# vincentfung13/MINE

Measured on AMD Instinct MI355X. Metric: train imgs/sec (whole node) RealEstate10K 384x256 N=64, higher is better.
Workload: dtype bf16; 1 GPU; model=monodepth2-resnet50-mpi, global_batch=4, seq_len=64, parallelism=dp1, img_h=256, img_w=384, n_planes=64

## Files before the change

mine_amd/ops/bn.py:

```python
from __future__ import annotations

import torch
import torch.nn as nn
import torch.nn.functional as F

from mine_amd.ops.backend import get_extension, is_deterministic

_ACT = {"none": 0, "relu": 1, "lrelu": 2, "elu": 3, "add_relu": 4}


class _BNActFn(torch.autograd.Function):
    @staticmethod
    def forward(ctx, x_flat, res_flat, mean, invstd, gamma, beta, M, C, act,
                sync):
        ext = get_extension(required=True)
        y = ext.bn_act_fwd(x_flat, res_flat, mean, invstd,
                           gamma, beta, M, C, act)
        ctx.save_for_backward(x_flat, res_flat, mean, invstd, gamma, beta)
        ctx.geom = (M, C, act, sync)
        ctx.det = is_deterministic()
        return y

    @staticmethod
    def backward(ctx, gy):
        ext = get_extension(required=True)
        x_flat, res_flat, mean, invstd, gamma, beta = ctx.saved_tensors
        M, C, act, sync = ctx.geom
        gy = gy.contiguous()
        red = ext.bn_act_bwd_reduce(x_flat, res_flat, gy, mean, invstd,
                                    gamma, beta, M, C, act, 0, ctx.det)
        dbeta, dgamma = red[:C], red[C:]
        M_norm = M
        if sync:
            dbeta, dgamma = dbeta.clone(), dgamma.clone()
            torch.distributed.all_reduce(red)
            M_norm = M * torch.distributed.get_world_size()
        dx, dres = ext.bn_act_bwd_dx(x_flat, res_flat, gy, mean, invstd,
                                     gamma, beta, red, M, C, act, M_norm)
        return (dx, dres if act == _ACT["add_relu"] else None, None, None,
                dgamma, dbeta, None, None, None, None)


class _JoinStatsFn(torch.autograd.Function):

    @staticmethod
    def forward(ctx, y_dec, y_base, bias, B, S):
        ext = get_extension(required=True)
        det = is_deterministic()
        _, K, H, W = y_dec.shape
        x_flat, sums = ext.bn_join_stats(
            y_dec.permute(0, 2, 3, 1).reshape(-1),
            y_base.permute(0, 2, 3, 1).reshape(-1),
            bias.contiguous(), B, S, H * W, K, 0, det)
        ctx.geom = (B, S, H, W, K)
        ctx.det = det
        ctx.mark_non_differentiable(sums)
        return x_flat.view(B * S, H, W, K).permute(0, 3, 1, 2), sums

    @staticmethod
    def backward(ctx, g, _gsums):
        B, S, H, W, K = ctx.geom
        g_nhwc = g.permute(0, 2, 3, 1)
        g_base = g_nhwc.reshape(B, S, H, W, K).sum(1).permute(0, 3, 1, 2)
        return g, g_base, g_nhwc.sum((1, 2)), None, None

# ... 43 lines not shown
    def forward(self, x: torch.Tensor, res: torch.Tensor = None,
                sums: torch.Tensor = None):
        assert (res is not None) == (self.act == "add_relu")
        use_kernel = (
            x.is_cuda and x.dim() == 4
            and x.dtype in (torch.float32, torch.bfloat16, torch.float16)
            and x.is_contiguous(memory_format=torch.channels_last)
            and (res is None or (res.dtype == x.dtype and res.is_contiguous(
                memory_format=torch.channels_last)))
            and (self.training or not torch.is_grad_enabled()))
        if not use_kernel:
            return self._fallback(x, res)

        ext = get_extension(required=True)
        B, C, H, W = x.shape
        M = B * H * W
        x_flat = x.permute(0, 2, 3, 1).reshape(-1)
        res_flat = res.permute(0, 2, 3, 1).reshape(-1) if res is not None \
            else torch.empty(0, device=x.device, dtype=x.dtype)

        do_sync = self.training and self.sync and \
            torch.distributed.is_initialized() and \
            torch.distributed.get_world_size() > 1
        if self.training:
            if self.num_batches_tracked is not None:
                self.num_batches_tracked.add_(1)
            mom = self.momentum if self.momentum is not None else \
                1.0 / float(self.num_batches_tracked)
            track = self.track_running_stats and self.running_mean is not None
            empty = torch.empty(0, device=x.device, dtype=torch.float32)
            if do_sync:
                if sums is None:
                    sums = ext.bn_sums(x_flat.detach(), M, C, 0,
                                       is_deterministic())
                torch.distributed.all_reduce(sums)
                Mg = M * torch.distributed.get_world_size()
                mean = sums[:C] / Mg
                var = (sums[C:] / Mg - mean * mean).clamp_min_(0.0)
                invstd = torch.rsqrt(var + self.eps)
                if track:
                    with torch.no_grad():
                        self.running_mean += mom * (mean - self.running_mean)
                        unbiased = var * Mg / max(Mg - 1, 1)
                        self.running_var += mom * (unbiased - self.running_var)
                mean = mean.contiguous()
                invstd = invstd.contiguous()
# ... 24 lines not shown
```

mine_amd/ops/csrc/bindings.hip:

```cpp

#include <torch/extension.h>
#include <ATen/hip/HIPContext.h>
#include <c10/hip/HIPException.h>
#include <hip/hip_runtime.h>

#include <algorithm>
#include <array>
#include <climits>
#include <string>
#include <vector>

#include "launchers.h"

namespace {

hipStream_t stream() {
  return at::hip::getCurrentHIPStreamMasqueradingAsCUDA().stream();
}


constexpr unsigned kF32 = 1u << kElemF32;
constexpr unsigned kBF16 = 1u << kElemBF16;
constexpr unsigned kF16 = 1u << kElemF16;
constexpr unsigned k16 = kBF16 | kF16;
// ... 595 lines not shown
  const auto scaled = M_norm != M ? red * ((double)M / (double)M_norm) : red;
  auto dx = at::empty_like(x);
  auto dres = add_relu ? at::empty_like(x) : at::empty({0}, x.options());
  launched(who, mine_bn_act_bwd_dx(
                    x.data_ptr(), add_relu ? res_p : nullptr, gy.data_ptr(),
                    mean.data_ptr<float>(), invstd.data_ptr<float>(),
                    gamma.data_ptr<float>(), beta.data_ptr<float>(),
                    scaled.data_ptr<float>(), dx.data_ptr(),
                    add_relu ? dres.data_ptr() : nullptr, M, (int)C, (int)act,
                    (int)max_blocks, elem_of(x.scalar_type(), who), stream()));
  return {dx, dres};
}

std::vector<at::Tensor> bn_act_bwd(at::Tensor x, at::Tensor res,
                                   at::Tensor gy, at::Tensor mean,
                                   at::Tensor invstd, at::Tensor gamma,
                                   at::Tensor beta, int64_t M, int64_t C,
                                   int64_t act, bool deterministic) {
  auto red = bn_act_bwd_reduce(x, res, gy, mean, invstd, gamma, beta,
                               M, C, act, 0, deterministic);
  auto dxr = bn_act_bwd_dx(x, res, gy, mean, invstd, gamma, beta, red,
                           M, C, act, M, 0);
  return {dxr[0], dxr[1], red.narrow(0, C, C), red.narrow(0, 0, C)};
}


at::Tensor mpi_head_fwd(at::Tensor z, int64_t N, bool alpha) {
  const char* who = "mpi_head_fwd";
  check_arg(who, "z", z, z, kFloat, N * 4);
  TORCH_CHECK(N > 0, who, ": N must be positive");
  auto out = at::empty({N * 4}, z.options().dtype(at::kFloat));
  launched(who, mine_mpi_head_fwd(z.data_ptr(), out.data_ptr<float>(), N,
                                  alpha ? 1 : 0, elem_of(z.scalar_type(), who),
                                  stream()));
  return out;
}

at::Tensor mpi_head_bwd(at::Tensor z, at::Tensor gout, int64_t N, bool alpha) {
  const char* who = "mpi_head_bwd";
  check_arg(who, "z", z, z, kFloat, N * 4);
  check_arg(who, "gout", gout, z, kF32, N * 4);
  TORCH_CHECK(N > 0, who, ": N must be positive");
  auto gz = at::empty_like(z);
  launched(who, mine_mpi_head_bwd(z.data_ptr(), gout.data_ptr<float>(),
                                  gz.data_ptr(), N, alpha ? 1 : 0,
                                  elem_of(z.scalar_type(), who), stream()));
// ... 378 lines not shown
  mod.def("bn_join_stats", &bn_join_stats,
          "x = (y_base + bias) + y_dec with its per-channel (sum, sumsq)",
          py::arg("y_dec"), py::arg("y_base"), py::arg("bias"), py::arg("B"),
          py::arg("S"), py::arg("HW"), py::arg("C"),
          py::arg("max_blocks") = 0, py::arg("deterministic") = false);
  mod.def("bn_act_fwd", &bn_act_fwd, "fused normalize + activation",
          py::arg("x"), py::arg("res"), py::arg("mean"), py::arg("invstd"),
          py::arg("gamma"), py::arg("beta"), py::arg("M"), py::arg("C"),
          py::arg("act"), py::arg("max_blocks") = 0);
  mod.def("bn_act_bwd", &bn_act_bwd,
          "fused BN+act backward -> dx, dres, dgamma, dbeta", py::arg("x"),
          py::arg("res"), py::arg("gy"), py::arg("mean"), py::arg("invstd"),
          py::arg("gamma"), py::arg("beta"), py::arg("M"), py::arg("C"),
          py::arg("act"), py::arg("deterministic") = false);
  mod.def("bn_act_bwd_reduce", &bn_act_bwd_reduce, py::arg("x"),
          py::arg("res"), py::arg("gy"), py::arg("mean"), py::arg("invstd"),
          py::arg("gamma"), py::arg("beta"), py::arg("M"), py::arg("C"),
          py::arg("act"), py::arg("max_blocks") = 0,
          py::arg("deterministic") = false);
  mod.def("bn_act_bwd_dx", &bn_act_bwd_dx, py::arg("x"), py::arg("res"),
          py::arg("gy"), py::arg("mean"), py::arg("invstd"), py::arg("gamma"),
          py::arg("beta"), py::arg("red"), py::arg("M"), py::arg("C"),
          py::arg("act"), py::arg("M_norm"), py::arg("max_blocks") = 0);
  mod.def("mpi_head_fwd", &mpi_head_fwd,
          "dispconv out -> packed fp32 MPI (sigmoid rgb, |x|+1e-4 sigma)");
  mod.def("mpi_head_bwd", &mpi_head_bwd);
  mod.def("conv3x3_fwd", &conv3x3_fwd,
          "fused reflect/zero-pad + 3x3 conv on MFMA 16x16x32 tiles",
          py::arg("x_flat"), py::arg("wp"), py::arg("bias"), py::arg("out"),
          py::arg("N"), py::arg("H"), py::arg("W"), py::arg("C"), py::arg("K"),
          py::arg("pad_mode"), py::arg("src_h"), py::arg("src_w"),
          py::arg("off"), py::arg("c_mem") = 0);
  mod.def("conv3x3_pack", &conv3x3_pack,
          "gather a conv weight into MFMA fragment order (bf16 or fp16)",
          py::arg("w_flat"), py::arg("lut"), py::arg("dtype") = py::none());
  mod.def("conv3x3_wrw", &conv3x3_wrw,
          "reflect-pad 3x3 conv weight gradient, fp32 (K, C, 3, 3)",
          py::arg("x_flat"), py::arg("gy_flat"), py::arg("N"), py::arg("H"),
          py::arg("W"), py::arg("C"), py::arg("K"), py::arg("max_slabs") = 0);
  mod.def("conv3x3_wrw_bias", &conv3x3_wrw_bias,
          "weight and bias gradient in one pass -> (dw, db)",
          py::arg("x_flat"), py::arg("gy_flat"), py::arg("N"), py::arg("H"),
          py::arg("W"), py::arg("C"), py::arg("K"), py::arg("max_slabs") = 0);
}
```

mine_amd/ops/csrc/bn_kernels.hip:

```cpp

#include <hip/hip_runtime.h>
#include <hip/hip_bf16.h>
#include <cstdint>

#include "launchers.h"

namespace {

constexpr int kBlock = 256;

enum Act : int { ACT_NONE = 0, ACT_RELU = 1, ACT_LRELU = 2, ACT_ELU = 3,
                 ACT_ADD_RELU = 4 };

template <int ACT>
__device__ __forceinline__ float act_fwd_t(float z) {
  if constexpr (ACT == ACT_RELU || ACT == ACT_ADD_RELU)
    return z > 0.0f ? z : 0.0f;
  else if constexpr (ACT == ACT_LRELU)
    return z > 0.0f ? z : 0.1f * z;
  else if constexpr (ACT == ACT_ELU)
    return z > 0.0f ? z : __expf(z) - 1.0f;
  else
    return z;
}
// ... 80 lines not shown
#pragma unroll
    for (int j = 0; j < V; ++j) {
      if constexpr (DET) {
        s_a[threadIdx.x * V + j] = a[j];
        s_b[threadIdx.x * V + j] = b[j];
      } else {
        atomicAdd(&s_a[lm.lane_cv * V + j], a[j]);
        atomicAdd(&s_b[lm.lane_cv * V + j], b[j]);
      }
    }
  }
  __syncthreads();
  if constexpr (DET) {
    det_block_flush(s_a, s_b, cgv * V, lm.rows_per_blk(), lm.ncv * V, out, C,
                    lm.c0v * V);
  } else {
    for (int i = threadIdx.x; i < lm.ncv * V; i += kBlock) {
      atomicAdd(&out[lm.c0v * V + i], s_a[i]);
      atomicAdd(&out[C + lm.c0v * V + i], s_b[i]);
    }
  }
}

template <typename T, int V, bool DET>
__global__ void __launch_bounds__(kBlock)
bn_stats_vec_kernel(const void* __restrict__ x, float* __restrict__ sums,
                    int64_t M, int C, int cgv) {
  using Vec = BnVec<T, V>;
  bn_reduce<V, DET, int>(
      C, cgv, sums, [&](const auto& lm, float (&acc)[V], float (&asq)[V]) {
        const int Cv = C / V;
        const Vec* xv = static_cast<const Vec*>(x);
        const int rstride = lm.rstride();
        for (int64_t m = lm.row0(); m < M; m += rstride) {
          const Vec val = xv[m * Cv + lm.col()];
#pragma unroll
          for (int j = 0; j < V; ++j) {
            const float f = (float)val.v[j];
            acc[j] += f;
            asq[j] += f * f;
          }
        }
      });
}

__device__ __forceinline__ void bn_finalize_channel(
    float sum, float sumsq, int c, float* __restrict__ mean,
    float* __restrict__ invstd, float* __restrict__ running_mean,
    float* __restrict__ running_var, int64_t M, float eps, float momentum) {
  const float mu = sum / (float)M;
  float var = sumsq / (float)M - mu * mu;
  var = var > 0.0f ? var : 0.0f;
  mean[c] = mu;
  invstd[c] = rsqrtf(var + eps);
  if (running_mean) {
    running_mean[c] += momentum * (mu - running_mean[c]);
    const float unbiased = M > 1 ? var * (float)M / (float)(M - 1) : var;
    running_var[c] += momentum * (unbiased - running_var[c]);
  }
}

__global__ void bn_finalize_kernel(const float* __restrict__ sums,
                                   float* __restrict__ mean,
                                   float* __restrict__ invstd,
                                   float* __restrict__ running_mean,
                                   float* __restrict__ running_var,
                                   int64_t M, int C, float eps,
                                   float momentum) {
  const int c = blockIdx.x * kBlock + threadIdx.x;
  if (c >= C) return;
  bn_finalize_channel(sums[c], sums[C + c], c, mean, invstd, running_mean,
                      running_var, M, eps, momentum);
}

__global__ void __launch_bounds__(kBlock)
bn_det_finish_kernel(const float* __restrict__ ws, int G, int C, int cw,
                     float* __restrict__ out, float* __restrict__ mean,
                     float* __restrict__ invstd,
                     float* __restrict__ running_mean,
                     float* __restrict__ running_var, int64_t M, float eps,
                     float momentum) {
  __shared__ float s_a[kBlock], s_b[kBlock];
// ... 22 lines not shown
    for (; g < G; g += np, row += step) {
      a += row[0];
      b += row[C];
    }
  }
  s_a[threadIdx.x] = a;
  s_b[threadIdx.x] = b;
  __syncthreads();
  if (threadIdx.x >= cw || c >= C) return;
  float ta = 0.0f, tb = 0.0f;
  for (int q = 0; q < np; ++q) {
    ta += s_a[q * cw + lane_c];
    tb += s_b[q * cw + lane_c];
  }
  if (out) {
    out[c] = ta;
    out[C + c] = tb;
  }
  if (mean)
    bn_finalize_channel(ta, tb, c, mean, invstd, running_mean, running_var, M,
                        eps, momentum);
}

template <typename T, int V, int ACT, bool DET>
__global__ void __launch_bounds__(kBlock)
bn_act_bwd_reduce_vec_kernel(const void* __restrict__ x,
                             const void* __restrict__ res,
                             const void* __restrict__ gy,
                             const float* __restrict__ mean,
                             const float* __restrict__ invstd,
                             const float* __restrict__ gamma,
                             const float* __restrict__ beta,
                             float* __restrict__ out,
                             int64_t M, int C, int cgv) {
  using Vec = BnVec<T, V>;
  bn_reduce<V, DET, int>(
      C, cgv, out, [&](const auto& lm, float (&db)[V], float (&dg)[V]) {
        const int Cv = C / V;
        const int cb = lm.col() * V;
        float mu[V], is[V], ga[V], be[V];
#pragma unroll
        for (int j = 0; j < V; ++j) {
          mu[j] = mean[cb + j];
          is[j] = invstd[cb + j];
          ga[j] = gamma[cb + j];
          be[j] = beta[cb + j];
        }
        const Vec* xv = static_cast<const Vec*>(x);
        const Vec* gv = static_cast<const Vec*>(gy);
        const Vec* rv = static_cast<const Vec*>(res);
        const int rstride = lm.rstride();
        for (int64_t m = lm.row0(); m < M; m += rstride) {
          const int64_t off = m * Cv + lm.col();
          const Vec xval = xv[off];
          const Vec gval = gv[off];
          Vec rval;
          if constexpr (ACT == ACT_ADD_RELU) rval = rv[off];
#pragma unroll
          for (int j = 0; j < V; ++j) {
            const float xh = ((float)xval.v[j] - mu[j]) * is[j];
            float z = xh * ga[j] + be[j];
            if constexpr (ACT == ACT_ADD_RELU) z += (float)rval.v[j];
            const float g = (float)gval.v[j] * act_grad_t<ACT>(z);
            db[j] += g;
            dg[j] += g * xh;
          }
        }
      });
}


template <typename T, int V, bool DET>
__global__ void __launch_bounds__(kBlock)
bn_join_stats_vec_kernel(const void* __restrict__ y_dec,
                         const void* __restrict__ y_base,
                         const void* __restrict__ bias, void* __restrict__ x,
                         float* __restrict__ sums,
                         int64_t M, int HW, int S, int C, int cgv) {
  using Vec = BnVec<T, V>;
  bn_reduce<V, DET, int64_t>(
      C, cgv, sums, [&](const auto& lm, float (&acc)[V], float (&asq)[V]) {
        const int Cv = C / V;
        const Vec* dv = static_cast<const Vec*>(y_dec) + lm.col();
        const Vec* bv = static_cast<const Vec*>(y_base) + lm.col();
        const Vec* pv = static_cast<const Vec*>(bias) + lm.col();
        Vec* xv = static_cast<Vec*>(x) + lm.col();
        const int64_t row0 = lm.row0();
        const int rstride = lm.rstride();
        const int dq = rstride / HW, dr = rstride % HW;
// ... 14 lines not shown
            out.v[j] = xo;
            const float f = (float)xo;
            acc[j] += f;
            asq[j] += f * f;
          }
          xv[m * Cv] = out;
          p += dr;
          const int carry = p >= HW ? 1 : 0;
          p -= carry ? HW : 0;
          bs += dq + carry;
          s += dq_s + carry;
          b += dq_b;
          if (s >= S) {
            s -= S;
            ++b;
          }
        }
      });
}


constexpr int fwd_unroll(int act) { return act == ACT_ADD_RELU ? 1 : 3; }
constexpr int dx_unroll(int act) { return act == ACT_ADD_RELU ? 1 : 2; }

template <typename T, int V, int ACT>
__device__ __forceinline__ BnVec<T, V> bn_fwd_vec(
    const BnVec<T, V>& xval, const BnVec<T, V>& rval, const float (&mu)[V],
    const float (&is)[V], const float (&ga)[V], const float (&be)[V]) {
  BnVec<T, V> out;
#pragma unroll
  for (int j = 0; j < V; ++j) {
    float z = ((float)xval.v[j] - mu[j]) * is[j] * ga[j] + be[j];
    if constexpr (ACT == ACT_ADD_RELU) z += (float)rval.v[j];
    out.v[j] = (T)act_fwd_t<ACT>(z);
  }
  return out;
}

template <typename T, int V, int ACT, int U>
__global__ void __launch_bounds__(kBlock)
bn_act_fwd_vec_kernel(const void* __restrict__ x, const void* __restrict__ res,
                      const float* __restrict__ mean,
                      const float* __restrict__ invstd,
                      const float* __restrict__ gamma,
                      const float* __restrict__ beta, void* __restrict__ y,
                      int64_t M, int C, int cgv) {
  using Vec = BnVec<T, V>;
  const int Cv = C / V;
  const LaneMap<int64_t, int64_t> lm(Cv, cgv);
  if (!lm.active()) return;
  const int cb = lm.col() * V;
  float mu[V], is[V], ga[V], be[V];
#pragma unroll
  for (int j = 0; j < V; ++j) {
    mu[j] = mean[cb + j];
    is[j] = invstd[cb + j];
    ga[j] = gamma[cb + j];
    be[j] = beta[cb + j];
  }
  const Vec* xv = static_cast<const Vec*>(x) + lm.col();
  const Vec* rv = static_cast<const Vec*>(res) + lm.col();
  Vec* yv = static_cast<Vec*>(y) + lm.col();
  const int64_t rstride = lm.rstride();
  const int64_t step = rstride * Cv;
  int64_t m = lm.row0();
  int64_t off = lm.row0() * Cv;
  for (; m + (U - 1) * rstride < M; m += U * rstride, off += U * step) {
    Vec xval[U], rval[U];
#pragma unroll
    for (int u = 0; u < U; ++u) xval[u] = xv[off + u * step];
    if constexpr (ACT == ACT_ADD_RELU) {
#pragma unroll
      for (int u = 0; u < U; ++u) rval[u] = rv[off + u * step];
    }
#pragma unroll
    for (int u = 0; u < U; ++u)
      yv[off + u * step] =
          bn_fwd_vec<T, V, ACT>(xval[u], rval[u], mu, is, ga, be);
  }
// ... 2 lines not shown
    Vec rval;
    if constexpr (ACT == ACT_ADD_RELU) rval = rv[off];
    yv[off] = bn_fwd_vec<T, V, ACT>(xval, rval, mu, is, ga, be);
  }
}

template <typename T, int V, int ACT>
__device__ __forceinline__ void bn_dx_vec(
    const BnVec<T, V>& xval, const BnVec<T, V>& rval, const BnVec<T, V>& gval,
    const float (&mu)[V], const float (&is)[V], const float (&ga)[V],
    const float (&be)[V], const float (&r0)[V], const float (&r1)[V],
    float invM, BnVec<T, V>& dxo, BnVec<T, V>& dro) {
#pragma unroll
  for (int j = 0; j < V; ++j) {
    const float xh = ((float)xval.v[j] - mu[j]) * is[j];
    float z = xh * ga[j] + be[j];
    if constexpr (ACT == ACT_ADD_RELU) z += (float)rval.v[j];
    const float g = (float)gval.v[j] * act_grad_t<ACT>(z);
    if constexpr (ACT == ACT_ADD_RELU) dro.v[j] = (T)g;
    dxo.v[j] = (T)(ga[j] * is[j] * (g - (r0[j] + xh * r1[j]) * invM));
  }
}

template <typename T, int V, int ACT, int U>
__global__ void __launch_bounds__(kBlock)
bn_act_bwd_dx_vec_kernel(const void* __restrict__ x,
                         const void* __restrict__ res,
                         const void* __restrict__ gy,
                         const float* __restrict__ mean,
                         const float* __restrict__ invstd,
                         const float* __restrict__ gamma,
                         const float* __restrict__ beta,
                         const float* __restrict__ red,
                         void* __restrict__ dx, void* __restrict__ dres,
                         int64_t M, int C, int cgv) {
  using Vec = BnVec<T, V>;
  const int Cv = C / V;
  const float invM = 1.0f / (float)M;
  const LaneMap<int64_t, int64_t> lm(Cv, cgv);
  if (!lm.active()) return;
  const int cb = lm.col() * V;
  float mu[V], is[V], ga[V], be[V], r0[V], r1[V];
#pragma unroll
  for (int j = 0; j < V; ++j) {
    mu[j] = mean[cb + j];
    is[j] = invstd[cb + j];
    ga[j] = gamma[cb + j];
    be[j] = beta[cb + j];
    r0[j] = red[cb + j];
    r1[j] = red[C + cb + j];
  }
  const Vec* xv = static_cast<const Vec*>(x) + lm.col();
  const Vec* rv = static_cast<const Vec*>(res) + lm.col();
  const Vec* gv = static_cast<const Vec*>(gy) + lm.col();
  Vec* dxv = static_cast<Vec*>(dx) + lm.col();
  Vec* drv = static_cast<Vec*>(dres) + lm.col();
  const int64_t rstride = lm.rstride();
  const int64_t step = rstride * Cv;
  int64_t m = lm.row0();
  int64_t off = lm.row0() * Cv;
  for (; m + (U - 1) * rstride < M; m += U * rstride, off += U * step) {
    Vec xval[U], gval[U], rval[U];
#pragma unroll
    for (int u = 0; u < U; ++u) {
      xval[u] = xv[off + u * step];
      gval[u] = gv[off + u * step];
    }
    if constexpr (ACT == ACT_ADD_RELU) {
#pragma unroll
      for (int u = 0; u < U; ++u) rval[u] = rv[off + u * step];
    }
#pragma unroll
    for (int u = 0; u < U; ++u) {
// ... 60 lines not shown
  BN_VEC_SWITCH(
      T, C, return (int)grid_rows_v(M, Cv, cgv, kMaxGridReduce, max_blocks).x)
}

template <typename T, bool DET>
void launch_bn_stats(const void* x, float* sums, int64_t M, int C,
                     int max_blocks, hipStream_t s) {
  BN_VEC_SWITCH(
      T, C,
      hipLaunchKernelGGL(
          (bn_stats_vec_kernel<T, V, DET>),
          grid_rows_v(M, Cv, cgv, kMaxGridReduce, max_blocks), dim3(kBlock), 0,
          s, x, sums, M, C, cgv))
}

template <typename T>
void launch_bn_act_fwd(const void* x, const void* res, const float* mean,
                       const float* invstd, const float* gamma,
                       const float* beta, void* y, int64_t M, int C, int act,
                       int max_blocks, hipStream_t s) {
#define BN_LAUNCH(A)                                                          \
  hipLaunchKernelGGL((bn_act_fwd_vec_kernel<T, V, A, fwd_unroll(A)>),         \
                     grid_rows_v(M, Cv, cgv, kMaxGridStream, max_blocks),     \
                     dim3(kBlock), 0, s, x, res, mean, invstd, gamma, beta, y, \
                     M, C, cgv)
  BN_VEC_SWITCH(T, C, BN_ACT_SWITCH(act, BN_LAUNCH))
#undef BN_LAUNCH
}

template <typename T, bool DET>
void launch_bn_act_bwd_reduce(const void* x, const void* res, const void* gy,
                              const float* mean, const float* invstd,
                              const float* gamma, const float* beta,
                              float* out, int64_t M, int C, int act,
                              int max_blocks, hipStream_t s) {
#define BN_LAUNCH(A)                                                       \
  hipLaunchKernelGGL((bn_act_bwd_reduce_vec_kernel<T, V, A, DET>),         \
                     grid_rows_v(M, Cv, cgv, kMaxGridReduce, max_blocks),  \
                     dim3(kBlock), 0, s, x, res, gy, mean, invstd, gamma,  \
                     beta, out, M, C, cgv)
  BN_VEC_SWITCH(T, C, BN_ACT_SWITCH(act, BN_LAUNCH))
#undef BN_LAUNCH
}

template <typename T>
void launch_bn_act_bwd_dx(const void* x, const void* res, const void* gy,
                          const float* mean, const float* invstd,
                          const float* gamma, const float* beta,
                          const float* red, void* dx, void* dres, int64_t M,
                          int C, int act, int max_blocks, hipStream_t s) {
#define BN_LAUNCH(A)                                                        \
  hipLaunchKernelGGL((bn_act_bwd_dx_vec_kernel<T, V, A, dx_unroll(A)>),     \
                     grid_rows_v(M, Cv, cgv, kMaxGridStream, max_blocks),   \
                     dim3(kBlock), 0, s, x, res, gy, mean, invstd, gamma,   \
                     beta, red, dx, dres, M, C, cgv)
  BN_VEC_SWITCH(T, C, BN_ACT_SWITCH(act, BN_LAUNCH))
#undef BN_LAUNCH
}

template <typename T, bool DET>
void launch_bn_join_stats(const void* y_dec, const void* y_base,
                          const void* bias, void* x, float* sums, int64_t M,
                          int HW, int S, int C, int max_blocks,
                          hipStream_t s) {
  BN_VEC_CASE(
      8, C,
      hipLaunchKernelGGL(
          (bn_join_stats_vec_kernel<T, V, DET>),
          grid_rows_v(M, Cv, cgv, kMaxGridReduce, max_blocks), dim3(kBlock), 0,
          s, y_dec, y_base, bias, x, sums, M, HW, S, C, cgv))
}

}

extern "C" int mine_bn_reduce_grid(int64_t M, int C, int max_blocks,
                                   int elem) {
  int grid = kNoKernel;
  MINE_ELEM_SWITCH(elem, grid = reduce_grid_x<T>(M, C, max_blocks))
  return grid;
}

extern "C" int mine_bn_stats(const void* x, float* sums, int64_t M, int C,
                             int max_blocks, int det, int elem,
                             hipStream_t s) {
  MINE_ELEM_SWITCH(
      elem, det ? launch_bn_stats<T, true>(x, sums, M, C, max_blocks, s)
                : launch_bn_stats<T, false>(x, sums, M, C, max_blocks, s))
  return kLaunched;
}

extern "C" int mine_bn_join_stats(const void* y_dec, const void* y_base,
                                  const void* bias, void* x, float* sums,
                                  int64_t M, int HW, int S, int C,
                                  int max_blocks, int det, int elem,
                                  hipStream_t s) {
// ... 69 lines not shown
```

mine_amd/ops/csrc/launchers.h:

```cpp
#pragma once

#include <hip/hip_runtime.h>

#include <cstdint>

constexpr int kElemF32 = 0;
constexpr int kElemBF16 = 1;
constexpr int kElemF16 = 2;

constexpr int kLaunched = 0;
constexpr int kNoKernel = -1;

#define MINE_ELEM_CASE(CODE, TYPE, ...) \
  case CODE: {                          \
    using T = TYPE;                     \
    __VA_ARGS__;                        \
  } break;
#define MINE_ELEM_SWITCH16(elem, ...)                      \
  switch (elem) {                                          \
    MINE_ELEM_CASE(kElemBF16, __hip_bfloat16, __VA_ARGS__) \
    MINE_ELEM_CASE(kElemF16, _Float16, __VA_ARGS__)        \
    default: return kNoKernel;                             \
  }
#define MINE_ELEM_SWITCH(elem, ...)                        \
// ... 69 lines not shown
                       void* x, float* sums, int64_t M, int HW, int S, int C,
                       int max_blocks, int det, int elem, hipStream_t s);
void mine_bn_det_finish(const float* ws, int G, int C, float* out, float* mean,
                        float* invstd, float* running_mean, float* running_var,
                        int64_t M, float eps, float momentum, hipStream_t s);
void mine_bn_finalize(const float* sums, float* mean, float* invstd,
                      float* running_mean, float* running_var, int64_t M,
                      int C, float eps, float momentum, hipStream_t s);
int mine_bn_act_fwd(const void* x, const void* res, const float* mean,
                    const float* invstd, const float* gamma, const float* beta,
                    void* y, int64_t M, int C, int act, int max_blocks,
                    int elem, hipStream_t s);
int mine_bn_act_bwd_reduce(const void* x, const void* res, const void* gy,
                           const float* mean, const float* invstd,
                           const float* gamma, const float* beta, float* out,
                           int64_t M, int C, int act, int max_blocks, int det,
                           int elem, hipStream_t s);
int mine_bn_act_bwd_dx(const void* x, const void* res, const void* gy,
                       const float* mean, const float* invstd,
                       const float* gamma, const float* beta, const float* red,
                       void* dx, void* dres, int64_t M, int C, int act,
                       int max_blocks, int elem, hipStream_t s);


int mine_mpi_head_fwd(const void* z, float* out, int64_t N, int alpha,
                      int elem, hipStream_t s);
int mine_mpi_head_bwd(const void* z, const float* gout, void* gz, int64_t N,
                      int alpha, int elem, hipStream_t s);


int mine_conv3x3_fwd(const void* x, const void* wp, const float* bias,
                     void* out, int N, int H, int W, int C, int c_mem, int K,
                     int pad_mode, int src_h, int src_w, int off, int elem,
                     hipStream_t stream);
int mine_conv3x3_pack(const void* w, int w_elem, const int64_t* lut, void* out,
                      int out_elem, int64_t n_out, int64_t n_w,
                      hipStream_t stream);


void mine_conv3x3_wrw_plan(int C, int Kmem, int64_t rows, int max_slabs,
                           int* slabs, int* nkb, int64_t* ws_floats);
int mine_conv3x3_wrw(const void* x, const void* gy, float* ws, float* dw,
                     float* db, int N, int H, int W, int C, int Kmem, int K,
                     int slabs, int elem, hipStream_t stream);


// ... 33 lines not shown
```

Before: 85.72 imgs/sec.

## Add two-launch compact BatchNorm path for small layers with fused finalize

For small BN layers (chosen by a size plan), forward now writes per-block partial sums and the activation kernel reduces them itself, finalizing mean, invstd and running stats inline. Backward likewise writes reduce partials and lets the dx kernel fold them. This cuts the kernel launches and finalize round-trips per BN layer, which matter when layers are small and launch-bound. The reduction loops also gain unrolled multi-row loads. Every consumer block redundantly re-reduces the partials, and the path is on by default through an env switch.

```diff
diff --git a/mine_amd/ops/bn.py b/mine_amd/ops/bn.py
--- a/mine_amd/ops/bn.py
+++ b/mine_amd/ops/bn.py
@@ -1,4 +1,6 @@
 from __future__ import annotations
+
+import os
 
 import torch
 import torch.nn as nn
@@ -41,6 +43,47 @@
                 dgamma, dbeta, None, None, None, None)
 
 
+def compact_enabled() -> bool:
+    return os.environ.get("MINE_BN_COMPACT", "1") != "0"
+
+
+_PLAN = {}
+
+
+def _plan_says_small(ext, M: int, C: int, dtype) -> bool:
+    key = (M, C, dtype)
+    if key not in _PLAN:
+        _PLAN[key] = bool(ext._bn.small_plan(M, C, dtype)[0])
+    return _PLAN[key]
+
+
+class _BNActSmallFn(torch.autograd.Function):
+
+    @staticmethod
+    def forward(ctx, x_flat, res_flat, gamma, beta, bufs, M, C, act, eps,
+                mom):
+        bn = get_extension(required=True)._bn
+        ws = bn.stats_partials(x_flat, M, C)
+        y, mean, invstd = bn.act_fwd_ws(x_flat, res_flat, ws, gamma, beta, M,
+                                        C, act, *bufs, eps, mom)
+        ctx.save_for_backward(x_flat, res_flat, mean, invstd, gamma, beta)
+        ctx.geom = (M, C, act)
+        return y
+
+    @staticmethod
+    def backward(ctx, gy):
+        bn = get_extension(required=True)._bn
+        x_flat, res_flat, mean, invstd, gamma, beta = ctx.saved_tensors
+        M, C, act = ctx.geom
+        gy = gy.contiguous()
+        ws = bn.bwd_reduce_partials(x_flat, res_flat, gy, mean, invstd, gamma,
+                                    beta, M, C, act)
+        dx, dres, red = bn.act_bwd_dx_ws(x_flat, res_flat, gy, mean, invstd,
+                                         gamma, beta, ws, M, C, act)
+        return (dx, dres if act == _ACT["add_relu"] else None, red[C:],
+                red[:C], None, None, None, None, None, None)
+
+
 class _JoinStatsFn(torch.autograd.Function):
 
     @staticmethod
@@ -130,6 +173,19 @@
         do_sync = self.training and self.sync and \
             torch.distributed.is_initialized() and \
             torch.distributed.get_world_size() > 1
+        if (self.training and not do_sync and sums is None
+                and self.momentum is not None and compact_enabled()
+                and _plan_says_small(ext, M, C, x.dtype)):
+            empty = torch.empty(0, device=x.device, dtype=torch.float32)
+            track = self.track_running_stats and self.running_mean is not None
+            nbt = self.num_batches_tracked
+            bufs = (self.running_mean if track else empty,
+                    self.running_var if track else empty,
+                    nbt if nbt is not None else empty)
+            y = _BNActSmallFn.apply(
+                x_flat, res_flat, self.weight.float(), self.bias.float(),
+                bufs, M, C, _ACT[self.act], self.eps, self.momentum)
+            return y.view(B, H, W, C).permute(0, 3, 1, 2)
         if self.training:
             if self.num_batches_tracked is not None:
                 self.num_batches_tracked.add_(1)
diff --git a/mine_amd/ops/csrc/bindings.hip b/mine_amd/ops/csrc/bindings.hip
--- a/mine_amd/ops/csrc/bindings.hip
+++ b/mine_amd/ops/csrc/bindings.hip
@@ -641,6 +641,134 @@
   auto dxr = bn_act_bwd_dx(x, res, gy, mean, invstd, gamma, beta, red,
                            M, C, act, M, 0);
   return {dxr[0], dxr[1], red.narrow(0, C, C), red.narrow(0, 0, C)};
+}
+
+struct BnSmall {
+  bool small;
+  int G, cgv, grid_x;
+};
+
+BnSmall bn_small(const char* who, const at::Tensor& x, int64_t M, int64_t C,
+                 int64_t max_blocks_reduce, int64_t max_blocks, int64_t cgv) {
+  for (const int64_t v : {max_blocks_reduce, max_blocks})
+    TORCH_CHECK(v >= 0 && v <= 4096, who, ": max_blocks out of range");
+  BnSmall p{};
+  const int rc = mine_bn_small_plan(M, (int)C, elem_of(x.scalar_type(), who),
+                                    &p.G, &p.cgv, &p.grid_x);
+  TORCH_CHECK(rc >= 0, who, ": no plan for this dtype");
+  p.small = rc == 1;
+  if (max_blocks_reduce > 0) p.G = (int)max_blocks_reduce;
+  if (max_blocks > 0) p.grid_x = (int)max_blocks;
+  if (cgv > 0) {
+    TORCH_CHECK(cgv <= 64 && (cgv & (cgv - 1)) == 0, who,
+                ": cgv must be a power of two up to 64");
+    p.cgv = (int)cgv;
+  }
+  return p;
+}
+
+std::tuple<bool, int64_t, int64_t, int64_t> bn_small_plan(
+    int64_t M, int64_t C, at::ScalarType dtype) {
+  const char* who = "small_plan";
+  check_ints(who, {M, C});
+  int G, cgv, grid_x;
+  const int rc = mine_bn_small_plan(M, (int)C, elem_of(dtype, who), &G, &cgv,
+                                    &grid_x);
+  return {rc == 1, G, cgv, grid_x};
+}
+
+at::Tensor bn_stats_partials(at::Tensor x, int64_t M, int64_t C,
+                             int64_t max_blocks, int64_t cgv) {
+  const char* who = "stats_partials";
+  check_bn_x(who, x, M, C, max_blocks);
+  const BnSmall p = bn_small(who, x, M, C, max_blocks, 0, cgv);
+  auto ws = at::empty({p.G, 2, C}, x.options().dtype(at::kFloat));
+  launched(who, mine_bn_stats_partials(x.data_ptr(), ws.data_ptr<float>(), M,
+                                       (int)C, p.G, p.cgv,
+                                       elem_of(x.scalar_type(), who),
+                                       stream()));
+  return ws;
+}
+
+std::vector<at::Tensor> bn_act_fwd_ws(
+    at::Tensor x, at::Tensor res, at::Tensor ws, at::Tensor gamma,
+    at::Tensor beta, int64_t M, int64_t C, int64_t act,
+    at::Tensor running_mean, at::Tensor running_var,
+    at::Tensor num_batches_tracked, double eps, double momentum,
+    int64_t max_blocks_reduce, int64_t max_blocks) {
+  const char* who = "act_fwd_ws";
+  check_bn_x(who, x, M, C, max_blocks);
+  const void* res_p = opt_arg<const void>(
+      who, "res", res, x, dtype_bit(x.scalar_type()), M * C);
+  const BnSmall p = bn_small(who, x, M, C, max_blocks_reduce, max_blocks, 0);
+  check_arg(who, "ws", ws, x, kF32, (int64_t)p.G * 2 * C);
+  check_arg(who, "gamma", gamma, x, kF32, C);
+  check_arg(who, "beta", beta, x, kF32, C);
+  TORCH_CHECK(act >= 0 && act <= 4, who, ": unknown activation");
+  TORCH_CHECK(act != 4 || res_p != nullptr, who,
+              ": res is required for add_relu");
+  float *rm, *rv;
+  check_running(who, x, running_mean, running_var, C, &rm, &rv);
+  int64_t* nbt = opt_arg<int64_t>(who, "num_batches_tracked",
+                                  num_batches_tracked, x, kI64, 1);
+  const auto fopt = x.options().dtype(at::kFloat);
+  auto y = at::empty_like(x);
+  auto mean = at::empty({C}, fopt);
+  auto invstd = at::empty({C}, fopt);
+  launched(who, mine_bn_act_fwd_ws(
+                    x.data_ptr(), act == 4 ? res_p : nullptr,
+                    ws.data_ptr<float>(), p.G, gamma.data_ptr<float>(),
+                    beta.data_ptr<float>(), y.data_ptr(),
+                    mean.data_ptr<float>(), invstd.data_ptr<float>(), rm, rv,
+                    nbt, M, (int)C, (int)act, p.grid_x, (float)eps,
+                    (float)momentum, elem_of(x.scalar_type(), who), stream()));
+  return {y, mean, invstd};
+}
+
+at::Tensor bn_bwd_reduce_partials(at::Tensor x, at::Tensor res, at::Tensor gy,
+                                  at::Tensor mean, at::Tensor invstd,
+                                  at::Tensor gamma, at::Tensor beta, int64_t M,
+                                  int64_t C, int64_t act, int64_t max_blocks,
+                                  int64_t cgv) {
+  const char* who = "bwd_reduce_partials";
+  const void* res_p = check_bn_act(who, x, res, mean, invstd, gamma, beta, M,
+                                   C, act, max_blocks);
+  check_arg(who, "gy", gy, x, dtype_bit(x.scalar_type()), M * C);
+  const BnSmall p = bn_small(who, x, M, C, max_blocks, 0, cgv);
+  auto ws = at::empty({p.G, 2, C}, x.options().dtype(at::kFloat));
+  launched(who, mine_bn_act_bwd_reduce_partials(
+                    x.data_ptr(), act == 4 ? res_p : nullptr, gy.data_ptr(),
+                    mean.data_ptr<float>(), invstd.data_ptr<float>(),
+                    gamma.data_ptr<float>(), beta.data_ptr<float>(),
+                    ws.data_ptr<float>(), M, (int)C, (int)act, p.G, p.cgv,
+                    elem_of(x.scalar_type(), who), stream()));
+  return ws;
+}
+
+std::vector<at::Tensor> bn_act_bwd_dx_ws(
+    at::Tensor x, at::Tensor res, at::Tensor gy, at::Tensor mean,
+    at::Tensor invstd, at::Tensor gamma, at::Tensor beta, at::Tensor ws,
+    int64_t M, int64_t C, int64_t act, int64_t max_blocks_reduce,
+    int64_t max_blocks) {
+  const char* who = "act_bwd_dx_ws";
+  const void* res_p = check_bn_act(who, x, res, mean, invstd, gamma, beta, M,
+                                   C, act, max_blocks);
+  check_arg(who, "gy", gy, x, dtype_bit(x.scalar_type()), M * C);
+  const BnSmall p = bn_small(who, x, M, C, max_blocks_reduce, max_blocks, 0);
+  check_arg(who, "ws", ws, x, kF32, (int64_t)p.G * 2 * C);
+  const bool add_relu = act == 4;
+  auto dx = at::empty_like(x);
+  auto dres = add_relu ? at::empty_like(x) : at::empty({0}, x.options());
+  auto red = at::empty({2 * C}, x.options().dtype(at::kFloat));
+  launched(who, mine_bn_act_bwd_dx_ws(
+                    x.data_ptr(), add_relu ? res_p : nullptr, gy.data_ptr(),
+                    mean.data_ptr<float>(), invstd.data_ptr<float>(),
+                    gamma.data_ptr<float>(), beta.data_ptr<float>(),
+                    ws.data_ptr<float>(), p.G, red.data_ptr<float>(),
+                    dx.data_ptr(), add_relu ? dres.data_ptr() : nullptr, M,
+                    (int)C, (int)act, p.grid_x, elem_of(x.scalar_type(), who),
+                    stream()));
+  return {dx, dres, red};
 }
 
 
@@ -1065,6 +1193,28 @@
           py::arg("gy"), py::arg("mean"), py::arg("invstd"), py::arg("gamma"),
           py::arg("beta"), py::arg("red"), py::arg("M"), py::arg("C"),
           py::arg("act"), py::arg("M_norm"), py::arg("max_blocks") = 0);
+  auto bn = mod.def_submodule(
+      "_bn", "two-launch BatchNorm for small layers: partials + consumer");
+  bn.def("small_plan", &bn_small_plan,
+         "(small, G, reduction cgv, consumer grid.x) for (M, C) of dtype",
+         py::arg("M"), py::arg("C"), py::arg("dtype"));
+  bn.def("stats_partials", &bn_stats_partials, py::arg("x"), py::arg("M"),
+         py::arg("C"), py::arg("max_blocks") = 0, py::arg("cgv") = 0);
+  bn.def("act_fwd_ws", &bn_act_fwd_ws, py::arg("x"), py::arg("res"),
+         py::arg("ws"), py::arg("gamma"), py::arg("beta"), py::arg("M"),
+         py::arg("C"), py::arg("act"), py::arg("running_mean"),
+         py::arg("running_var"), py::arg("num_batches_tracked"),
+         py::arg("eps"), py::arg("momentum"),
+         py::arg("max_blocks_reduce") = 0, py::arg("max_blocks") = 0);
+  bn.def("bwd_reduce_partials", &bn_bwd_reduce_partials, py::arg("x"),
+         py::arg("res"), py::arg("gy"), py::arg("mean"), py::arg("invstd"),
+         py::arg("gamma"), py::arg("beta"), py::arg("M"), py::arg("C"),
+         py::arg("act"), py::arg("max_blocks") = 0, py::arg("cgv") = 0);
+  bn.def("act_bwd_dx_ws", &bn_act_bwd_dx_ws, py::arg("x"), py::arg("res"),
+         py::arg("gy"), py::arg("mean"), py::arg("invstd"), py::arg("gamma"),
+         py::arg("beta"), py::arg("ws"), py::arg("M"), py::arg("C"),
+         py::arg("act"), py::arg("max_blocks_reduce") = 0,
+         py::arg("max_blocks") = 0);
   mod.def("mpi_head_fwd", &mpi_head_fwd,
           "dispconv out -> packed fp32 MPI (sigmoid rgb, |x|+1e-4 sigma)");
   mod.def("mpi_head_bwd", &mpi_head_bwd);
diff --git a/mine_amd/ops/csrc/bn_kernels.hip b/mine_amd/ops/csrc/bn_kernels.hip
--- a/mine_amd/ops/csrc/bn_kernels.hip
+++ b/mine_amd/ops/csrc/bn_kernels.hip
@@ -126,7 +126,7 @@
   }
 }
 
-template <typename T, int V, bool DET>
+template <typename T, int V, bool DET, int U = 1>
 __global__ void __launch_bounds__(kBlock)
 bn_stats_vec_kernel(const void* __restrict__ x, float* __restrict__ sums,
                     int64_t M, int C, int cgv) {
@@ -136,7 +136,25 @@
         const int Cv = C / V;
         const Vec* xv = static_cast<const Vec*>(x);
         const int rstride = lm.rstride();
-        for (int64_t m = lm.row0(); m < M; m += rstride) {
+        int64_t m = lm.row0();
+        if constexpr (U > 1) {
+          for (; m + (int64_t)(U - 1) * rstride < M; m += (int64_t)U * rstride) {
+            Vec val[U];
+#pragma unroll
+            for (int u = 0; u < U; ++u)
+              val[u] = xv[(m + (int64_t)u * rstride) * Cv + lm.col()];
+#pragma unroll
+            for (int u = 0; u < U; ++u) {
+#pragma unroll
+              for (int j = 0; j < V; ++j) {
+                const float f = (float)val[u].v[j];
+                acc[j] += f;
+                asq[j] += f * f;
+              }
+            }
+          }
+        }
+        for (; m < M; m += rstride) {
           const Vec val = xv[m * Cv + lm.col()];
 #pragma unroll
           for (int j = 0; j < V; ++j) {
@@ -148,20 +166,37 @@
       });
 }
 
+struct BnMoments {
+  float mu, var, invstd;
+};
+__device__ __forceinline__ BnMoments bn_moments(float sum, float sumsq,
+                                                int64_t M, float eps) {
+  const float mu = sum / (float)M;
+  float var = sumsq / (float)M - mu * mu;
+  var = var > 0.0f ? var : 0.0f;
+  return {mu, var, rsqrtf(var + eps)};
+}
+
+__device__ __forceinline__ void bn_store_channel(
+    const BnMoments& mo, int c, float* __restrict__ mean,
+    float* __restrict__ invstd, float* __restrict__ running_mean,
+    float* __restrict__ running_var, int64_t M, float momentum) {
+  mean[c] = mo.mu;
+  invstd[c] = mo.invstd;
+  if (running_mean) {
+    running_mean[c] += momentum * (mo.mu - running_mean[c]);
+    const float unbiased =
+        M > 1 ? mo.var * (float)M / (float)(M - 1) : mo.var;
+    running_var[c] += momentum * (unbiased - running_var[c]);
+  }
+}
+
 __device__ __forceinline__ void bn_finalize_channel(
     float sum, float sumsq, int c, float* __restrict__ mean,
     float* __restrict__ invstd, float* __restrict__ running_mean,
     float* __restrict__ running_var, int64_t M, float eps, float momentum) {
-  const float mu = sum / (float)M;
-  float var = sumsq / (float)M - mu * mu;
-  var = var > 0.0f ? var : 0.0f;
-  mean[c] = mu;
-  invstd[c] = rsqrtf(var + eps);
-  if (running_mean) {
-    running_mean[c] += momentum * (mu - running_mean[c]);
-    const float unbiased = M > 1 ? var * (float)M / (float)(M - 1) : var;
-    running_var[c] += momentum * (unbiased - running_var[c]);
-  }
+  bn_store_channel(bn_moments(sum, sumsq, M, eps), c, mean, invstd,
+                   running_mean, running_var, M, momentum);
 }
 
 __global__ void bn_finalize_kernel(const float* __restrict__ sums,
@@ -230,7 +265,7 @@
                         eps, momentum);
 }
 
-template <typename T, int V, int ACT, bool DET>
+template <typename T, int V, int ACT, bool DET, int U = 1>
 __global__ void __launch_bounds__(kBlock)
 bn_act_bwd_reduce_vec_kernel(const void* __restrict__ x,
                              const void* __restrict__ res,
@@ -258,12 +293,7 @@
         const Vec* gv = static_cast<const Vec*>(gy);
         const Vec* rv = static_cast<const Vec*>(res);
         const int rstride = lm.rstride();
-        for (int64_t m = lm.row0(); m < M; m += rstride) {
-          const int64_t off = m * Cv + lm.col();
-          const Vec xval = xv[off];
-          const Vec gval = gv[off];
-          Vec rval;
-          if constexpr (ACT == ACT_ADD_RELU) rval = rv[off];
+        auto add_row = [&](const Vec& xval, const Vec& rval, const Vec& gval) {
 #pragma unroll
           for (int j = 0; j < V; ++j) {
             const float xh = ((float)xval.v[j] - mu[j]) * is[j];
@@ -273,6 +303,29 @@
             db[j] += g;
             dg[j] += g * xh;
           }
+        };
+        int64_t m = lm.row0();
+        if constexpr (U > 1) {
+          for (; m + (int64_t)(U - 1) * rstride < M; m += (int64_t)U * rstride) {
+            Vec xval[U], gval[U], rval[U];
+#pragma unroll
+            for (int u = 0; u < U; ++u) {
+              const int64_t off = (m + (int64_t)u * rstride) * Cv + lm.col();
+              xval[u] = xv[off];
+              gval[u] = gv[off];
+              if constexpr (ACT == ACT_ADD_RELU) rval[u] = rv[off];
+            }
+#pragma unroll
+            for (int u = 0; u < U; ++u) add_row(xval[u], rval[u], gval[u]);
+          }
+        }
+        for (; m < M; m += rstride) {
+          const int64_t off = m * Cv + lm.col();
+          const Vec xval = xv[off];
+          const Vec gval = gv[off];
+          Vec rval;
+          if constexpr (ACT == ACT_ADD_RELU) rval = rv[off];
+          add_row(xval, rval, gval);
         }
       });
 }
@@ -333,6 +386,64 @@
 
 constexpr int fwd_unroll(int act) { return act == ACT_ADD_RELU ? 1 : 3; }
 constexpr int dx_unroll(int act) { return act == ACT_ADD_RELU ? 1 : 2; }
+constexpr int red_unroll(int act) { return act == ACT_ADD_RELU ? 2 : 4; }
+
+template <bool WS>
+struct BnFwdStats {
+  const float* __restrict__ mean;
+  const float* __restrict__ invstd;
+};
+template <>
+struct BnFwdStats<true> {
+  const float* __restrict__ ws;
+  int G;
+  float* __restrict__ mean;
+  float* __restrict__ invstd;
+  float* __restrict__ running_mean;
+  float* __restrict__ running_var;
+  int64_t* __restrict__ num_batches_tracked;
+  float eps, momentum;
+};
+template <bool WS>
+struct BnBwdSums {
+  const float* __restrict__ red;
+};
+template <>
+struct BnBwdSums<true> {
+  const float* __restrict__ ws;
+  int G;
+  float* __restrict__ red;
+};
+
+__device__ __forceinline__ float ws_sum(const float* __restrict__ p, int G,
+                                        int64_t step) {
+  float t = 0.0f;
+  int g = 0;
+  for (; g + 7 < G; g += 8, p += 8 * step) {
+    float v[8];
+#pragma unroll
+    for (int u = 0; u < 8; ++u) v[u] = p[u * step];
+#pragma unroll
+    for (int u = 0; u < 8; ++u) t += v[u];
+  }
+  for (; g < G; ++g, p += step) t += *p;
+  return t;
+}
+
+template <int V, typename LM>
+__device__ __forceinline__ void ws_prologue(const LM& lm,
+                                            const float* __restrict__ ws,
+                                            int G, int C,
+                                            float (&s)[2 * 64 * V]) {
+  const int nch = lm.ncv * V;
+  const float* base = ws + lm.c0v * V;
+  for (int i = threadIdx.x; i < 2 * nch; i += kBlock) {
+    const int which = i >= nch ? 1 : 0;
+    const int ci = i - which * nch;
+    s[which * 64 * V + ci] = ws_sum(base + which * C + ci, G, 2 * (int64_t)C);
+  }
+  __syncthreads();
+}
 
 template <typename T, int V, int ACT>
 __device__ __forceinline__ BnVec<T, V> bn_fwd_vec(
@@ -348,24 +459,46 @@
   return out;
 }
 
-template <typename T, int V, int ACT, int U>
+template <typename T, int V, int ACT, int U, bool WS = false>
 __global__ void __launch_bounds__(kBlock)
 bn_act_fwd_vec_kernel(const void* __restrict__ x, const void* __restrict__ res,
-                      const float* __restrict__ mean,
-                      const float* __restrict__ invstd,
+                      const BnFwdStats<WS> st,
                       const float* __restrict__ gamma,
                       const float* __restrict__ beta, void* __restrict__ y,
                       int64_t M, int C, int cgv) {
   using Vec = BnVec<T, V>;
   const int Cv = C / V;
   const LaneMap<int64_t, int64_t> lm(Cv, cgv);
-  if (!lm.active()) return;
+  float mu[V], is[V], ga[V], be[V];
+  if constexpr (WS) {
+    __shared__ float s_sum[2 * 64 * V];
+    ws_prologue<V>(lm, st.ws, st.G, C, s_sum);
+    if (!lm.active()) return;
+    const bool owner = blockIdx.x == 0 && threadIdx.x < cgv;
+#pragma unroll
+    for (int j = 0; j < V; ++j) {
+      const int cl = lm.lane_cv * V + j;
+      const BnMoments mo =
+          bn_moments(s_sum[cl], s_sum[64 * V + cl], M, st.eps);
+      mu[j] = mo.mu;
+      is[j] = mo.invstd;
+      if (owner)
+        bn_store_channel(mo, lm.col() * V + j, st.mean, st.invstd,
+                         st.running_mean, st.running_var, M, st.momentum);
+    }
+    if (owner && blockIdx.y == 0 && threadIdx.x == 0 &&
+        st.num_batches_tracked)
+      *st.num_batches_tracked += 1;
+  } else {
+    if (!lm.active()) return;
+  }
   const int cb = lm.col() * V;
-  float mu[V], is[V], ga[V], be[V];
 #pragma unroll
   for (int j = 0; j < V; ++j) {
-    mu[j] = mean[cb + j];
-    is[j] = invstd[cb + j];
+    if constexpr (!WS) {
+      mu[j] = st.mean[cb + j];
+      is[j] = st.invstd[cb + j];
+    }
     ga[j] = gamma[cb + j];
     be[j] = beta[cb + j];
   }
@@ -414,7 +547,7 @@
   }
 }
 
-template <typename T, int V, int ACT, int U>
+template <typename T, int V, int ACT, int U, bool WS = false>
 __global__ void __launch_bounds__(kBlock)
 bn_act_bwd_dx_vec_kernel(const void* __restrict__ x,
                          const void* __restrict__ res,
@@ -423,24 +556,43 @@
                          const float* __restrict__ invstd,
                          const float* __restrict__ gamma,
                          const float* __restrict__ beta,
-                         const float* __restrict__ red,
+                         const BnBwdSums<WS> sums,
                          void* __restrict__ dx, void* __restrict__ dres,
                          int64_t M, int C, int cgv) {
   using Vec = BnVec<T, V>;
   const int Cv = C / V;
   const float invM = 1.0f / (float)M;
   const LaneMap<int64_t, int64_t> lm(Cv, cgv);
-  if (!lm.active()) return;
+  float mu[V], is[V], ga[V], be[V], r0[V], r1[V];
+  if constexpr (WS) {
+    __shared__ float s_sum[2 * 64 * V];
+    ws_prologue<V>(lm, sums.ws, sums.G, C, s_sum);
+    if (!lm.active()) return;
+    const bool owner = blockIdx.x == 0 && threadIdx.x < cgv;
+#pragma unroll
+    for (int j = 0; j < V; ++j) {
+      const int cl = lm.lane_cv * V + j;
+      r0[j] = s_sum[cl];
+      r1[j] = s_sum[64 * V + cl];
+      if (owner) {
+        sums.red[lm.col() * V + j] = r0[j];
+        sums.red[C + lm.col() * V + j] = r1[j];
+      }
+    }
+  } else {
+    if (!lm.active()) return;
+  }
   const int cb = lm.col() * V;
-  float mu[V], is[V], ga[V], be[V], r0[V], r1[V];
 #pragma unroll
   for (int j = 0; j < V; ++j) {
     mu[j] = mean[cb + j];
     is[j] = invstd[cb + j];
     ga[j] = gamma[cb + j];
     be[j] = beta[cb + j];
-    r0[j] = red[cb + j];
-    r1[j] = red[C + cb + j];
+    if constexpr (!WS) {
+      r0[j] = sums.red[cb + j];
+      r1[j] = sums.red[C + cb + j];
+    }
   }
   const Vec* xv = static_cast<const Vec*>(x) + lm.col();
   const Vec* rv = static_cast<const Vec*>(res) + lm.col();
@@ -547,8 +699,9 @@
 #define BN_LAUNCH(A)                                                          \
   hipLaunchKernelGGL((bn_act_fwd_vec_kernel<T, V, A, fwd_unroll(A)>),         \
                      grid_rows_v(M, Cv, cgv, kMaxGridStream, max_blocks),     \
-                     dim3(kBlock), 0, s, x, res, mean, invstd, gamma, beta, y, \
-                     M, C, cgv)
+                     dim3(kBlock), 0, s, x, res,                              \
+                     BnFwdStats<false>{mean, invstd}, gamma, beta, y, M, C,   \
+                     cgv)
   BN_VEC_SWITCH(T, C, BN_ACT_SWITCH(act, BN_LAUNCH))
 #undef BN_LAUNCH
 }
@@ -578,7 +731,7 @@
   hipLaunchKernelGGL((bn_act_bwd_dx_vec_kernel<T, V, A, dx_unroll(A)>),     \
                      grid_rows_v(M, Cv, cgv, kMaxGridStream, max_blocks),   \
                      dim3(kBlock), 0, s, x, res, gy, mean, invstd, gamma,   \
-                     beta, red, dx, dres, M, C, cgv)
+                     beta, BnBwdSums<false>{red}, dx, dres, M, C, cgv)
   BN_VEC_SWITCH(T, C, BN_ACT_SWITCH(act, BN_LAUNCH))
 #undef BN_LAUNCH
 }
@@ -596,6 +749,167 @@
           s, y_dec, y_base, bias, x, sums, M, HW, S, C, cgv))
 }
 
+
+constexpr int kSmallRows = 4;
+constexpr int kSmallMaxConsumers = 1024;
+constexpr int kSmallPrologueBytes = 32 << 10;
+constexpr int64_t kSmallWideBytes = (int64_t)8 << 20;
+constexpr int kSmallMinCgv = 4;
+constexpr int64_t kSmallMaxBytes = (int64_t)16 << 20;
+constexpr int kSmallMaxG = 4096;
+
+struct BnSmallPlan {
+  bool small;
+  int G, cgv, grid_x;
+};
+
+inline int64_t ceil_div(int64_t a, int64_t b) { return (a + b - 1) / b; }
+
+template <typename T>
+BnSmallPlan small_plan(int64_t M, int C) {
+  BN_VEC_SWITCH(T, C, {
+    const int64_t bytes = M * C * (int64_t)sizeof(T);
+    const int nch = (Cv < cgv ? Cv : cgv) * V;
+    const int budget =
+        kSmallPrologueBytes * (bytes >= kSmallWideBytes ? 2 : 1);
+    int G = budget / (8 * nch);
+    G = G < 1 ? 1 : G;
+    int rc = cgv < kSmallMinCgv ? cgv : kSmallMinCgv;
+    while (rc < cgv && M < (int64_t)G * (kBlock / rc)) rc <<= 1;
+    while (G > 1 && M < (int64_t)G * (kBlock / rc)) G >>= 1;
+    int64_t consumers = ceil_div(M * Cv, (int64_t)kBlock * kSmallRows);
+    consumers = consumers < kSmallMaxConsumers ? consumers : kSmallMaxConsumers;
+    const int64_t gx = consumers / ceil_div(Cv, cgv);
+    return BnSmallPlan{bytes <= kSmallMaxBytes, G, rc,
+                       (int)(gx < 1 ? 1 : gx)};
+  })
+}
+
+template <typename T>
+void launch_bn_stats_partials(const void* x, float* ws, int64_t M, int C,
+                              int G, int cgv_r, hipStream_t s) {
+  BN_VEC_SWITCH(
+      T, C,
+      hipLaunchKernelGGL((bn_stats_vec_kernel<T, V, true, 4>),
+                         dim3(G, (Cv + cgv_r - 1) / cgv_r), dim3(kBlock), 0, s,
+                         x, ws, M, C, cgv_r))
+}
+
+template <typename T>
+void launch_bn_act_fwd_ws(const void* x, const void* res,
+                          const BnFwdStats<true>& st, const float* gamma,
+                          const float* beta, void* y, int64_t M, int C,
+                          int act, int grid_x, hipStream_t s) {
+#define BN_LAUNCH(A)                                                       \
+  hipLaunchKernelGGL((bn_act_fwd_vec_kernel<T, V, A, fwd_unroll(A), true>), \
+                     dim3(grid_x, (Cv + cgv - 1) / cgv), dim3(kBlock), 0, s, \
+                     x, res, st, gamma, beta, y, M, C, cgv)
+  BN_VEC_SWITCH(T, C, BN_ACT_SWITCH(act, BN_LAUNCH))
+#undef BN_LAUNCH
+}
+
+template <typename T>
+void launch_bn_act_bwd_reduce_partials(const void* x, const void* res,
+                                       const void* gy, const float* mean,
+                                       const float* invstd,
+                                       const float* gamma, const float* beta,
+                                       float* ws, int64_t M, int C, int act,
+                                       int G, int cgv_r, hipStream_t s) {
+#define BN_LAUNCH(A)                                                         \
+  hipLaunchKernelGGL(                                                        \
+      (bn_act_bwd_reduce_vec_kernel<T, V, A, true, red_unroll(A)>),          \
+      dim3(G, (Cv + cgv_r - 1) / cgv_r), dim3(kBlock), 0, s, x, res, gy,     \
+      mean, invstd, gamma, beta, ws, M, C, cgv_r)
+  BN_VEC_SWITCH(T, C, BN_ACT_SWITCH(act, BN_LAUNCH))
+#undef BN_LAUNCH
+}
+
+template <typename T>
+void launch_bn_act_bwd_dx_ws(const void* x, const void* res, const void* gy,
+                             const float* mean, const float* invstd,
+                             const float* gamma, const float* beta,
+                             const BnBwdSums<true>& sums, void* dx, void* dres,
+                             int64_t M, int C, int act, int grid_x,
+                             hipStream_t s) {
+#define BN_LAUNCH(A)                                                          \
+  hipLaunchKernelGGL(                                                         \
+      (bn_act_bwd_dx_vec_kernel<T, V, A, dx_unroll(A), true>),                \
+      dim3(grid_x, (Cv + cgv - 1) / cgv), dim3(kBlock), 0, s, x, res, gy,     \
+      mean, invstd, gamma, beta, sums, dx, dres, M, C, cgv)
+  BN_VEC_SWITCH(T, C, BN_ACT_SWITCH(act, BN_LAUNCH))
+#undef BN_LAUNCH
+}
+
+inline bool valid_cgv(int cgv) {
+  return cgv >= 1 && cgv <= 64 && (cgv & (cgv - 1)) == 0;
+}
+inline bool valid_grid(int g) { return g >= 1 && g <= kSmallMaxG; }
+inline bool valid_chunks(int C, int cgv) { return C / cgv < 65535; }
+
+}
+
+extern "C" int mine_bn_small_plan(int64_t M, int C, int elem, int* G, int* cgv,
+                                  int* grid_x) {
+  BnSmallPlan p{};
+  MINE_ELEM_SWITCH(elem, p = small_plan<T>(M, C))
+  *G = p.G;
+  *cgv = p.cgv;
+  *grid_x = p.grid_x;
+  return p.small ? 1 : 0;
+}
+
+extern "C" int mine_bn_stats_partials(const void* x, float* ws, int64_t M,
+                                      int C, int G, int cgv, int elem,
+                                      hipStream_t s) {
+  if (!valid_grid(G) || !valid_cgv(cgv) || !valid_chunks(C, cgv))
+    return kNoKernel;
+  MINE_ELEM_SWITCH(elem, launch_bn_stats_partials<T>(x, ws, M, C, G, cgv, s))
+  return kLaunched;
+}
+
+extern "C" int mine_bn_act_fwd_ws(const void* x, const void* res,
+                                  const float* ws, int G, const float* gamma,
+                                  const float* beta, void* y, float* mean,
+                                  float* invstd, float* running_mean,
+                                  float* running_var,
+                                  int64_t* num_batches_tracked, int64_t M,
+                                  int C, int act, int grid_x, float eps,
+                                  float momentum, int elem, hipStream_t s) {
+  if (!valid_grid(G) || !valid_grid(grid_x)) return kNoKernel;
+  const BnFwdStats<true> st{ws,           G,           mean,
+                            invstd,       running_mean, running_var,
+                            num_batches_tracked, eps,  momentum};
+  MINE_ELEM_SWITCH(elem, launch_bn_act_fwd_ws<T>(x, res, st, gamma, beta, y, M,
+                                                 C, act, grid_x, s))
+  return kLaunched;
+}
+
+extern "C" int mine_bn_act_bwd_reduce_partials(
+    const void* x, const void* res, const void* gy, const float* mean,
+    const float* invstd, const float* gamma, const float* beta, float* ws,
+    int64_t M, int C, int act, int G, int cgv, int elem, hipStream_t s) {
+  if (!valid_grid(G) || !valid_cgv(cgv) || !valid_chunks(C, cgv))
+    return kNoKernel;
+  MINE_ELEM_SWITCH(elem, launch_bn_act_bwd_reduce_partials<T>(
+                             x, res, gy, mean, invstd, gamma, beta, ws, M, C,
+                             act, G, cgv, s))
+  return kLaunched;
+}
+
+extern "C" int mine_bn_act_bwd_dx_ws(const void* x, const void* res,
+                                     const void* gy, const float* mean,
+                                     const float* invstd, const float* gamma,
+                                     const float* beta, const float* ws, int G,
+                                     float* red, void* dx, void* dres,
+                                     int64_t M, int C, int act, int grid_x,
+                                     int elem, hipStream_t s) {
+  if (!valid_grid(G) || !valid_grid(grid_x)) return kNoKernel;
+  const BnBwdSums<true> sums{ws, G, red};
+  MINE_ELEM_SWITCH(elem, launch_bn_act_bwd_dx_ws<T>(x, res, gy, mean, invstd,
+                                                    gamma, beta, sums, dx,
+                                                    dres, M, C, act, grid_x,
+                                                    s))
+  return kLaunched;
 }
 
 extern "C" int mine_bn_reduce_grid(int64_t M, int C, int max_blocks,
diff --git a/mine_amd/ops/csrc/launchers.h b/mine_amd/ops/csrc/launchers.h
--- a/mine_amd/ops/csrc/launchers.h
+++ b/mine_amd/ops/csrc/launchers.h
@@ -115,6 +115,29 @@
                        void* dx, void* dres, int64_t M, int C, int act,
                        int max_blocks, int elem, hipStream_t s);
 
+int mine_bn_small_plan(int64_t M, int C, int elem, int* G, int* cgv,
+                       int* grid_x);
+int mine_bn_stats_partials(const void* x, float* ws, int64_t M, int C, int G,
+                           int cgv, int elem, hipStream_t s);
+int mine_bn_act_fwd_ws(const void* x, const void* res, const float* ws, int G,
+                       const float* gamma, const float* beta, void* y,
+                       float* mean, float* invstd, float* running_mean,
+                       float* running_var, int64_t* num_batches_tracked,
+                       int64_t M, int C, int act, int grid_x, float eps,
+                       float momentum, int elem, hipStream_t s);
+int mine_bn_act_bwd_reduce_partials(const void* x, const void* res,
+                                    const void* gy, const float* mean,
+                                    const float* invstd, const float* gamma,
+                                    const float* beta, float* ws, int64_t M,
+                                    int C, int act, int G, int cgv, int elem,
+                                    hipStream_t s);
+int mine_bn_act_bwd_dx_ws(const void* x, const void* res, const void* gy,
+                          const float* mean, const float* invstd,
+                          const float* gamma, const float* beta,
+                          const float* ws, int G, float* red, void* dx,
+                          void* dres, int64_t M, int C, int act, int grid_x,
+                          int elem, hipStream_t s);
+
 
 int mine_mpi_head_fwd(const void* z, float* out, int64_t N, int alpha,
                       int elem, hipStream_t s);
```

After: 92.85 imgs/sec, median of 6. 1.08x the previous value.
